# Arcadia-Science/arcadia-microscopy-tools

Measured on AMD Instinct MI355X. Metric: fields-of-view/sec (4x2048^2 uint16) end-to-end segment+props, higher is better.
Workload: dtype f64; 1 GPU; configs[2]: synthetic 4-channel 2048x2048 uint16 FOVs, DAPI Gaussian+Otsu+open/close+EDT+peak markers+watershed nuclei (SEEDED relief, seeds_first: marker pixels spread first in raster order, cannot tie; SURVEY A.8's plain -EDT relief with exact ties is reported under sublines.a8_exact) + clear_border/relabel + morphology and 4-channel intensity regionprops; mode=weak scaling, 192 FOVs per GPU per step, streams_per_gpu=4, fovs_per_launch=48, max_cells_per_fov=2048, distinct_fovs_per_gpu=8, resident_in_hbm=True

## Files before the change

arcadia_microscopy_tools_amd/_thresholds.py:

```python
from __future__ import annotations

import numpy as np
from scipy import ndimage as ndi


def counts_centers_u16(hist65536: np.ndarray):
    nz = np.flatnonzero(hist65536)
    lo, hi = int(nz[0]), int(nz[-1])
    return hist65536[lo:hi + 1].astype(np.int64), np.arange(lo, hi + 1)


def counts_centers_f64(hist: np.ndarray, vmin: float, vmax: float):
    edges = np.linspace(vmin, vmax, len(hist) + 1)
    return hist.astype(np.int64), (edges[:-1] + edges[1:]) / 2.0


def otsu(counts, bin_centers):
    counts = counts.astype(float)
    if len(bin_centers) == 1:
        return bin_centers[0]
    w_lo = np.cumsum(counts)
    w_hi = np.cumsum(counts[::-1])[::-1]
    weighted = counts * bin_centers
    m_lo = np.cumsum(weighted) / w_lo
# ... 52 lines not shown
    length = peak_height * x1 - width * y1
    arg_level = np.argmax(length) + arg_low_level
    if flip:
        arg_level = nbins - arg_level - 1
    return bin_centers[arg_level]


def minimum(counts, bin_centers, max_iter: int = 10000):

    def local_maxima(h):
        step = np.diff(h)
        nz = np.flatnonzero(step)
        if nz.size == 0:
            return []
        falling = step[nz] < 0
        prev_rising = np.ones(nz.size, bool)
        prev_rising[1:] = ~falling[:-1]
        return nz[falling & prev_rising].tolist()

    smooth = counts.astype(np.float64, copy=False)
    maxima: list[int] = []
    counter = 0
    for counter in range(max_iter):
        smooth = ndi.uniform_filter1d(smooth, 3)
        maxima = local_maxima(smooth)
        if len(maxima) < 3:
            break
    if len(maxima) != 2:
        raise RuntimeError("Unable to find two maxima in histogram")
    elif counter == max_iter - 1:
        raise RuntimeError("Maximum iteration reached for histogram smoothing")
    k = np.argmin(smooth[maxima[0]:maxima[1] + 1])
    return bin_centers[maxima[0] + k]


def mean_from_hist(counts, values):
    return float(np.sum(counts * values)) / float(np.sum(counts))


def li_from_hist(counts, values, tolerance=None, initial_guess=None, wrap_dtype=None):
    values = values.astype(np.int64)
    counts = np.asarray(counts)
    image_min = int(values[0])
    v = values - image_min
    if wrap_dtype is not None and np.dtype(wrap_dtype).kind == "i" and int(v[-1]) > int(np.iinfo(wrap_dtype).max):
        half = int(np.iinfo(wrap_dtype).max) + 1
        v = (v + half) % (2 * half) - half
        order = np.argsort(v, kind="stable")
        v, counts = v[order], counts[order]
    present = v[counts > 0]
    if present.size == 1:
        return values[0]
    tolerance = tolerance or np.min(np.diff(present)) / 2
    total_sum = np.sum(counts * v)
    total_cnt = np.sum(counts)
    t_next = total_sum / total_cnt if initial_guess is None else initial_guess - image_min
    t_curr = -2 * tolerance
    csum = np.cumsum(counts * v)
    ccnt = np.cumsum(counts)
    with np.errstate(invalid="ignore", divide="ignore"):
        while abs(t_next - t_curr) > tolerance:
            t_curr = t_next
            k = int(np.searchsorted(v, t_curr, side="right")) - 1
            s_le = csum[k] if k >= 0 else 0
            c_le = ccnt[k] if k >= 0 else 0
            mean_back = np.float64(s_le) / np.float64(c_le)
            mean_fore = np.float64(total_sum - s_le) / np.float64(total_cnt - c_le)
            t_next = (mean_back - mean_fore) / (np.log(mean_back) - np.log(mean_fore))
    return t_next + image_min


def prefix_rule(v: np.ndarray, vmin: float, vmax: float, nbins: int = 256):
    v = np.ascontiguousarray(v, dtype=np.float64)
    if (v < 0).any():
        raise ValueError("the prefix order holds for non-negative samples only")
    hi32 = v.view(np.uint64) >> np.uint64(32) << np.uint64(32)
    vlo, vhi = hi32.view(np.float64), (hi32 | np.uint64(0xFFFFFFFF)).view(np.float64)
    edges = np.linspace(vmin, vmax, nbins + 1)
    bins = np.clip(np.searchsorted(edges, vlo, side="right") - 1, 0, nbins - 1)
    centres = (edges[:-1] + edges[1:]) / 2.0
    above = vlo > centres[bins]
    undecided = ((bins < nbins - 1) & (vhi >= edges[bins + 1])) | (~above & (vhi > centres[bins]))
    return bins, above, undecided
```

arcadia_microscopy_tools_amd/csrc/amt_filters.hip:

```cpp
#include "amt_internal.h"

template <typename TIn>
__device__ __forceinline__ double load_as_f64(const TIn* p, size_t i, double scale);
template <>
__device__ __forceinline__ double load_as_f64<uint16_t>(const uint16_t* p, size_t i, double scale) {
    return (double)p[i] * scale;
}
template <>
__device__ __forceinline__ double load_as_f64<double>(const double* p, size_t i, double scale) {
    return p[i];
}

template <typename TIn>
__device__ __forceinline__ double cvt_f64(TIn v, double scale);
template <>
__device__ __forceinline__ double cvt_f64<uint16_t>(uint16_t v, double scale) {
    return (double)v * scale;
}
template <>
__device__ __forceinline__ double cvt_f64<double>(double v, double scale) {
    return v;
}

template <typename F>
// ... 879 lines not shown

__global__ void convert_u16_f64_kernel(const uint16_t* __restrict__ in, double scale, double* __restrict__ out,
                                       size_t n) {
    size_t i = (size_t)blockIdx.x * blockDim.x + threadIdx.x;
    size_t stride = (size_t)gridDim.x * blockDim.x;
    for (; i < n; i += stride) out[i] = (double)in[i] * scale;
}

__global__ void copy_f64_kernel(const double* __restrict__ in, double* __restrict__ out, size_t n) {
    size_t i = (size_t)blockIdx.x * blockDim.x + threadIdx.x;
    size_t stride = (size_t)gridDim.x * blockDim.x;
    for (; i < n; i += stride) out[i] = in[i];
}

extern "C" int amt_convert_u16_f64(amt_ctx* ctx, const uint16_t* in, double scale, double* out, size_t n) {
    AMT_TRY(amt_set_device(ctx));
    AMT_REQUIRE(in && out, "convert_u16_f64: null pointer");
    if (n == 0) return AMT_OK;
    hipLaunchKernelGGL(convert_u16_f64_kernel, dim3(amt_grid_for(n, 256)), dim3(256), 0, ctx->stream, in, scale, out,
                       n);
    AMT_LAUNCH_CHECK();
    return AMT_OK;
}

extern "C" int amt_gaussian(amt_ctx* ctx, const void* in, int in_dtype, double scale, double* out, int nplanes, int H,
                            int W, const double* weights, int radius, int mode, double cval, size_t in_plane_stride,
                            double* minmax_dev) {
    AMT_TRY(amt_set_device(ctx));
    AMT_TRY(check_gauss_args(in, in_dtype, out, nplanes, H, W, weights, radius));
    AMT_REQUIRE(in_plane_stride == 0 || in_plane_stride >= (size_t)H * W, "gaussian: in_plane_stride smaller than a plane");
    AMT_REQUIRE(radius > 0 || in_plane_stride == 0 || in_plane_stride == (size_t)H * W,
                "gaussian: strided input needs radius >= 1");
    if (nplanes == 0) return AMT_OK;
    size_t n = (size_t)nplanes * H * W;
    if (radius == 0) {
        if (in_dtype == AMT_U16) {
            AMT_TRY(amt_convert_u16_f64(ctx, (const uint16_t*)in, scale, out, n));
        } else {
            hipLaunchKernelGGL(copy_f64_kernel, dim3(amt_grid_for(n, 256)), dim3(256), 0, ctx->stream,
                               (const double*)in, out, n);
            AMT_LAUNCH_CHECK();
        }
        if (minmax_dev) {
            amt_scratch s(ctx);
            amt_buf<unsigned long long> keys(s, (size_t)2 * nplanes);
            AMT_TRY(s.commit());
            AMT_TRY(amt_i_minmax_f64(ctx, out, keys, minmax_dev, nplanes, (size_t)H * W));
        }
        return AMT_OK;
    }
    amt_scratch s(ctx);
    amt_buf<double> wdev(s, 2 * radius + 1);
    amt_buf<double> tmp(s, n, radius > FR_MAX);
    amt_buf<unsigned long long> keys(s, (size_t)2 * nplanes, minmax_dev != nullptr);
    AMT_TRY(s.commit());
    AMT_TRY(amt_param_upload(ctx, wdev, weights, (2 * radius + 1) * sizeof(double)));
    if (!minmax_dev)
        return gaussian_dispatch(ctx, in, in_dtype, scale, out, tmp, nplanes, H, W, wdev, radius, mode, cval,
                                 in_plane_stride);
    if (radius > FR_MAX) {
        AMT_TRY(gaussian_dispatch(ctx, in, in_dtype, scale, out, tmp, nplanes, H, W, wdev, radius, mode, cval,
                                  in_plane_stride));
        return amt_i_minmax_f64(ctx, out, keys, minmax_dev, nplanes, (size_t)H * W);
    }
    AMT_TRY(amt_i_minmax_init(ctx, keys, nplanes));
    AMT_TRY(gaussian_dispatch(ctx, in, in_dtype, scale, out, tmp, nplanes, H, W, wdev, radius, mode, cval,
                              in_plane_stride, keys));
    return amt_i_minmax_finish(ctx, keys, minmax_dev, nplanes);
}


__device__ __forceinline__ double gl_edge(double lo, double hi, double step, int i) {
    return i == GL_NBINS ? hi : (double)i * step + lo;
}

__device__ __forceinline__ int gl_bin(double v, double lo, double hi, double step, double norm) {
    int b = (int)((v - lo) * norm);
    b = b < 0 ? 0 : (b > GL_NBINS - 1 ? GL_NBINS - 1 : b);
    while (b > 0 && v < gl_edge(lo, hi, step, b)) --b;
    while (b < GL_NBINS - 1 && v >= gl_edge(lo, hi, step, b + 1)) ++b;
    return b;
}

__global__ void __launch_bounds__(256) prefix_codes_kernel(const uint32_t* __restrict__ prefix,
                                                           const double* __restrict__ minmax,
                                                           uint32_t* __restrict__ hist, uint16_t* __restrict__ codes,
                                                           size_t n, uint32_t* __restrict__ und_count,
                                                           uint32_t* __restrict__ und_list) {
    __shared__ uint32_t lh[4 * GL_NBINS];
    const int plane = blockIdx.y;
    const int lane = threadIdx.x & 63;
    const double lo = minmax[2 * plane], hi = minmax[2 * plane + 1];
    const uint32_t* src = prefix + (size_t)plane * n;
    uint16_t* dst = codes + (size_t)plane * n;
    const size_t first = ((size_t)blockIdx.x * 256 + threadIdx.x) * 4, stride = (size_t)gridDim.x * 1024;
    if (!(lo < hi)) {
        for (size_t i0 = first; i0 < n; i0 += stride) *reinterpret_cast<uint2*>(dst + i0) = make_uint2(0u, 0u);
        return;
    }
    for (int i = threadIdx.x; i < 4 * GL_NBINS; i += 256) lh[i] = 0;
    __syncthreads();
    uint32_t* mine = lh + (threadIdx.x >> 6) * GL_NBINS;
    const double step = (hi - lo) / (double)GL_NBINS, norm = (double)GL_NBINS / (hi - lo);
    uint32_t* cnt = und_count + (size_t)plane * PFX_CNT_STRIDE;
    uint32_t* list = und_list + (size_t)plane * PFX_CAP;
    bool dead = false;
    for (size_t i0 = first; i0 < n && !dead; i0 += stride) {
        const uint4 p4 = *reinterpret_cast<const uint4*>(src + i0);
        const unsigned p[4] = {p4.x, p4.y, p4.z, p4.w};
        int b4[4];
        double elo4[4], ehi4[4];
#pragma unroll
        for (int u = 0; u < 4; ++u) {
            const double vlo = __hiloint2double((int)p[u], 0);
            int b = (int)((vlo - lo) * norm);
            b = b < 0 ? 0 : (b > GL_NBINS - 1 ? GL_NBINS - 1 : b);
            b4[u] = b;
            elo4[u] = (double)b * step + lo;
            ehi4[u] = gl_edge(lo, hi, step, b + 1);
        }
        unsigned cd[4], undm = 0;
#pragma unroll
        for (int u = 0; u < 4; ++u) {
            const double vlo = __hiloint2double((int)p[u], 0), vhi = __hiloint2double((int)p[u], (int)0xffffffffu);
            int b = b4[u];
            if (vlo < elo4[u] || (b < GL_NBINS - 1 && vlo >= ehi4[u])) {
                b = gl_bin(vlo, lo, hi, step, norm);
                elo4[u] = gl_edge(lo, hi, step, b);
                ehi4[u] = gl_edge(lo, hi, step, b + 1);
            }
            const double ctr = (elo4[u] + ehi4[u]) / 2.0;
            const bool gt = vlo > ctr;
            const bool und = (b < GL_NBINS - 1 && vhi >= ehi4[u]) || (!gt && vhi > ctr);
            undm |= (und ? 1u : 0u) << u;
            cd[u] = und ? 0u : (((unsigned)b << 1) | (gt ? 1u : 0u));
            const unsigned long long act = __ballot(!und);
            if (!act) continue;
            const int l0 = __ffsll((long long)act) - 1;
            const int b0 = __shfl(b, l0);
            const unsigned long long s0 = __ballot(!und && b == b0);
            if (lane == l0) atomicAdd(&mine[b0], (unsigned)__popcll(s0));
            unsigned long long rest = act & ~s0;
            if (rest) {
                const int l1 = __ffsll((long long)rest) - 1;
                const int b1 = __shfl(b, l1);
                const unsigned long long s1 = __ballot(!und && b == b1);
                if (lane == l1) atomicAdd(&mine[b1], (unsigned)__popcll(s1));
                rest &= ~s1;
                if ((rest >> lane) & 1ull) atomicAdd(&mine[b], 1u);
            }
        }
        *reinterpret_cast<uint2*>(dst + i0) = make_uint2(cd[0] | (cd[1] << 16), cd[2] | (cd[3] << 16));
        const unsigned long long any = __ballot(undm != 0);
        if (any) {
            const unsigned long long m0 = __ballot(undm & 1u), m1 = __ballot(undm & 2u), m2 = __ballot(undm & 4u),
                                     m3 = __ballot(undm & 8u);
            const unsigned n0 = __popcll(m0), n1 = __popcll(m1), n2 = __popcll(m2), n3 = __popcll(m3);
            const int leader = __ffsll((long long)any) - 1;
            unsigned base = 0;
            if (lane == leader) base = atomicAdd(cnt, n0 + n1 + n2 + n3);
            base = __shfl(base, leader);
            const unsigned long long below = (1ull << lane) - 1ull;
            const unsigned pos[4] = {base + (unsigned)__popcll(m0 & below), base + n0 + (unsigned)__popcll(m1 & below),
                                     base + n0 + n1 + (unsigned)__popcll(m2 & below),
                                     base + n0 + n1 + n2 + (unsigned)__popcll(m3 & below)};
#pragma unroll
            for (int u = 0; u < 4; ++u)
                if (((undm >> u) & 1u) && pos[u] < PFX_CAP) list[pos[u]] = (uint32_t)(i0 + u);
            dead = base + n0 + n1 + n2 + n3 > PFX_CAP;
        }
    }
    __syncthreads();
    uint32_t* gh = hist + (size_t)plane * GL_NBINS;
    for (int i = threadIdx.x; i < GL_NBINS; i += 256) {
        const uint32_t c = lh[i] + lh[GL_NBINS + i] + lh[2 * GL_NBINS + i] + lh[3 * GL_NBINS + i];
        if (c) atomicAdd(&gh[i], c);
    }
}

constexpr int PFX_FIX_BLOCKS = 64;
template <int R>
__global__ void __launch_bounds__(64) prefix_fixup_kernel(const uint16_t* __restrict__ in, double scale, int H, int W,
                                                          const double* __restrict__ wts, int mode, size_t in_stride,
                                                          const double* __restrict__ minmax,
                                                          const uint32_t* __restrict__ und_count,
                                                          const uint32_t* __restrict__ und_list,
                                                          uint32_t* __restrict__ hist, uint16_t* __restrict__ codes) {
    constexpr int K = 2 * R + 1;
    static_assert(K <= 32, "one half wave per sample");
    __shared__ double cs[2][32];
    const int plane = blockIdx.y;
    const uint32_t cnt = und_count[(size_t)plane * PFX_CNT_STRIDE];
    uint32_t* gh = hist + (size_t)plane * GL_NBINS;
    if (cnt > PFX_CAP) {
        if (blockIdx.x == 0)
            for (int i = threadIdx.x; i < GL_NBINS; i += 64) gh[i] = 0;
        return;
    }
    if (blockIdx.x * 2u >= cnt) return;
    double w[R + 1];
#pragma unroll
    for (int j = 0; j <= R; ++j) w[j] = wts[R - j];
    const uint16_t* src = in + (size_t)plane * in_stride;
    const double lo = minmax[2 * plane], hi = minmax[2 * plane + 1];
    const double step = (hi - lo) / (double)GL_NBINS, norm = (double)GL_NBINS / (hi - lo);
    const int half = threadIdx.x >> 5, d = threadIdx.x & 31;
    for (uint32_t e0 = blockIdx.x * 2u; e0 < cnt; e0 += 2u * PFX_FIX_BLOCKS) {
        const bool valid = e0 + half < cnt;
        const uint32_t idx = valid ? und_list[(size_t)plane * PFX_CAP + e0 + half] : 0u;
        const int y = (int)(idx / (uint32_t)W), x = (int)(idx % (uint32_t)W);
        if (valid && d < K) cs[half][d] = gauss_column<R>(src, scale, H, W, mode, y, x - R + d, w);
        __syncthreads();
        if (valid && d == 0) {
            double c[K];
#pragma unroll
            for (int k = 0; k < K; ++k) c[k] = cs[half][k];
            const double v = gauss_taps<R>(&c[R], w);
            const int b = gl_bin(v, lo, hi, step, norm);
            const double ctr = (gl_edge(lo, hi, step, b) + gl_edge(lo, hi, step, b + 1)) / 2.0;
            atomicAdd(&gh[b], 1u);
            codes[(size_t)plane * H * W + idx] = (uint16_t)((b << 1) | (v > ctr ? 1 : 0));
        }
        __syncthreads();
    }
}

template <int R>
static int launch_codes(amt_ctx* ctx, const uint16_t* in, double scale, int nplanes, int H, int W, const double* wdev,
                        int mode, size_t in_stride, unsigned long long* keys, double* mm, uint32_t* hist,
                        uint16_t* codes, uint32_t* prefix, uint32_t* und_count, uint32_t* und_list) {
    constexpr int RP = (R + 7) & ~7;
    constexpr int OUTW2 = 256 - 2 * RP;
    const int gx2 = (W + OUTW2 - 1) / OUTW2;
    int TH2 = 256;
    while (TH2 > 32 && (long long)gx2 * ((H + TH2 - 1) / TH2) * nplanes < 4LL * ctx->num_cus) TH2 >>= 1;
    dim3 grid2(gx2, (H + TH2 - 1) / TH2, nplanes);
    AMT_TRY(amt_i_minmax_init(ctx, keys, nplanes));
    if (prefix) {
        hipLaunchKernelGGL((gauss_lds_kernel<R, 3>), grid2, dim3(256), 0, ctx->stream, in, scale, (double*)nullptr, H, W,
                           wdev, mode, in_stride, TH2, keys, (const double*)nullptr, (uint32_t*)nullptr,
                           (uint16_t*)nullptr, prefix, (const uint32_t*)nullptr);
        AMT_LAUNCH_CHECK();
        AMT_TRY(amt_i_minmax_finish(ctx, keys, mm, nplanes));
        AMT_HIP_CHECK(hipMemsetAsync(hist, 0, (size_t)nplanes * GL_NBINS * sizeof(uint32_t), ctx->stream));
        AMT_HIP_CHECK(hipMemsetAsync(und_count, 0, (size_t)nplanes * PFX_CNT_STRIDE * sizeof(uint32_t), ctx->stream));
        const size_t n = (size_t)H * W;
        hipLaunchKernelGGL(prefix_codes_kernel, dim3(amt_grid_for(n, 256 * 16, 512), nplanes), dim3(256), 0, ctx->stream,
                           (const uint32_t*)prefix, (const double*)mm, hist, codes, n, und_count, und_list);
        AMT_LAUNCH_CHECK();
        hipLaunchKernelGGL((prefix_fixup_kernel<R>), dim3(PFX_FIX_BLOCKS, nplanes), dim3(64), 0, ctx->stream, in, scale, H, W,
                           wdev, mode, in_stride, (const double*)mm, (const uint32_t*)und_count,
                           (const uint32_t*)und_list, hist, codes);
        AMT_LAUNCH_CHECK();
        hipLaunchKernelGGL((gauss_lds_kernel<R, 2>), grid2, dim3(256), 0, ctx->stream, in, scale, (double*)nullptr, H, W,
                           wdev, mode, in_stride, TH2, (unsigned long long*)nullptr, (const double*)mm, hist, codes,
                           (uint32_t*)nullptr, (const uint32_t*)und_count);
        AMT_LAUNCH_CHECK();
        return AMT_OK;
    }
    hipLaunchKernelGGL((gauss_lds_kernel<R, 1>), grid2, dim3(256), 0, ctx->stream, in, scale, (double*)nullptr, H, W,
                       wdev, mode, in_stride, TH2, keys, (const double*)nullptr, (uint32_t*)nullptr, (uint16_t*)nullptr,
                       (uint32_t*)nullptr, (const uint32_t*)nullptr);
    AMT_LAUNCH_CHECK();
    AMT_TRY(amt_i_minmax_finish(ctx, keys, mm, nplanes));
    AMT_HIP_CHECK(hipMemsetAsync(hist, 0, (size_t)nplanes * GL_NBINS * sizeof(uint32_t), ctx->stream));
    hipLaunchKernelGGL((gauss_lds_kernel<R, 2>), grid2, dim3(256), 0, ctx->stream, in, scale, (double*)nullptr, H, W,
                       wdev, mode, in_stride, TH2, (unsigned long long*)nullptr, (const double*)mm, hist, codes,
                       (uint32_t*)nullptr, (const uint32_t*)nullptr);
    AMT_LAUNCH_CHECK();
    return AMT_OK;
}

extern "C" int amt_gaussian_otsu_codes_supported(int H, int W, int radius, int mode, size_t in_plane_stride) {
    const bool modeok = mode == AMT_MODE_NEAREST || mode == AMT_MODE_REFLECT || mode == AMT_MODE_MIRROR;
    return radius >= 1 && radius <= FR_MAX && modeok && W % 8 == 0 && W >= 256 && H > 2 * radius &&
           (in_plane_stride == 0 || in_plane_stride % 8 == 0);
}

extern "C" int amt_gaussian_otsu_codes(amt_ctx* ctx, const uint16_t* in, double scale, int nplanes, int H, int W,
                                       const double* weights, int radius, int mode, size_t in_plane_stride,
                                       double* minmax_dev, uint32_t* hist_dev, double* thr_dev, double* thr_code_dev,
                                       uint16_t* codes, uint32_t* prefix) {
    AMT_TRY(amt_set_device(ctx));
    AMT_REQUIRE(in && weights && minmax_dev && hist_dev && thr_dev && thr_code_dev && codes && nplanes >= 0,
                "gaussian_otsu_codes: bad arguments");
    AMT_REQUIRE(amt_gaussian_otsu_codes_supported(H, W, radius, mode, in_plane_stride) &&
                    (reinterpret_cast<uintptr_t>(in) & 15) == 0 && (reinterpret_cast<uintptr_t>(codes) & 15) == 0 &&
                    (reinterpret_cast<uintptr_t>(prefix) & 15) == 0,
                "gaussian_otsu_codes: unsupported shape / radius / mode / alignment (ask "
                "amt_gaussian_otsu_codes_supported; the separate operators handle every case)");
    if (nplanes == 0) return AMT_OK;
    if (in_plane_stride == 0) in_plane_stride = (size_t)H * W;
    bool ordered = scale > 0.0 && (size_t)H * W <= 0xffffffffull;
    for (int i = 0; i <= 2 * radius; ++i) ordered = ordered && weights[i] >= 0.0;
    if (!ordered) prefix = nullptr;
    amt_scratch s(ctx);
    amt_buf<double> wdev(s, 2 * radius + 1);
    amt_buf<unsigned long long> keys(s, (size_t)2 * nplanes);
    amt_buf<uint32_t> und_count(s, (size_t)nplanes * PFX_CNT_STRIDE, prefix != nullptr);
    amt_buf<uint32_t> und_list(s, (size_t)nplanes * PFX_CAP, prefix != nullptr);
    AMT_TRY(s.commit());
    AMT_TRY(amt_param_upload(ctx, wdev, weights, (2 * radius + 1) * sizeof(double)));
    switch (radius) {
#define AMT_CODES_CASE(RR)                                                                                            \
    case RR:                                                                                                          \
        AMT_TRY(launch_codes<RR>(ctx, in, scale, nplanes, H, W, wdev, mode, in_plane_stride, keys, minmax_dev, hist_dev, \
                                 codes, prefix, und_count, und_list));                                                \
        break;
        AMT_CODES_CASE(1)
        AMT_CODES_CASE(2)
        AMT_CODES_CASE(3)
        AMT_CODES_CASE(4)
        AMT_CODES_CASE(5)
        AMT_CODES_CASE(6)
        AMT_CODES_CASE(7)
        AMT_CODES_CASE(8)
        AMT_CODES_CASE(9)
        AMT_CODES_CASE(10)
        AMT_CODES_CASE(11)
        AMT_CODES_CASE(12)
#undef AMT_CODES_CASE
        default:
            amt_set_error("gaussian_otsu_codes: radius %d", radius);
            return AMT_EINVAL;
    }
    return amt_i_otsu_from_hist(ctx, hist_dev, minmax_dev, GL_NBINS, thr_dev, thr_code_dev, nplanes);
}

__global__ void sub_inplace_kernel(double* __restrict__ a, const double* __restrict__ b, size_t n) {
    size_t i = (size_t)blockIdx.x * blockDim.x + threadIdx.x;
    size_t stride = (size_t)gridDim.x * blockDim.x;
    for (; i < n; i += stride) a[i] = a[i] - b[i];
}

extern "C" int amt_convolve_axis0(amt_ctx* ctx, const void* in, int in_dtype, double scale, double* out, int nplanes, int L,
                                  int inner, const double* weights, int radius, int mode, double cval) {
    AMT_TRY(amt_set_device(ctx));
    AMT_TRY(check_gauss_args(in, in_dtype, out, nplanes, L, inner, weights, radius));
    AMT_REQUIRE(radius >= 1, "convolve_axis0: radius must be >= 1");
    AMT_REQUIRE((const void*)in != (const void*)out, "convolve_axis0: in-place operation is not supported");
    if (nplanes == 0) return AMT_OK;
    const int r = radius;
// ... 232 lines not shown
```

arcadia_microscopy_tools_amd/csrc/amt_internal.h:

```cpp
#pragma once
#include "amt_common.h"

#include <type_traits>

template <int ITEMS>
__global__ void __launch_bounds__(1024) amt_scan_excl_kernel(int* __restrict__ data, int len, size_t plane_stride,
                                                             int* __restrict__ total,
                                                             const int* __restrict__ len_dev = nullptr) {
    __shared__ int s[1024];
    __shared__ int carry;
    int* d = data + (size_t)blockIdx.x * plane_stride;
    if (len_dev) len = len_dev[blockIdx.x];
    if (threadIdx.x == 0) carry = 0;
    __syncthreads();
    for (int start = 0; start < len; start += 1024 * ITEMS) {
        const int b = start + threadIdx.x * ITEMS;
        int v[ITEMS];
        int sum = 0;
#pragma unroll
        for (int k = 0; k < ITEMS; ++k) {
            v[k] = (b + k < len) ? d[b + k] : 0;
            sum += v[k];
        }
        s[threadIdx.x] = sum;
        __syncthreads();
        for (int off = 1; off < 1024; off <<= 1) {
            int t = threadIdx.x >= off ? s[threadIdx.x - off] : 0;
            __syncthreads();
            s[threadIdx.x] += t;
            __syncthreads();
        }
        const int c = carry;
        int run = c + s[threadIdx.x] - sum;
#pragma unroll
        for (int k = 0; k < ITEMS; ++k) {
            if (b + k < len) d[b + k] = run;
            run += v[k];
        }
        __syncthreads();
        if (threadIdx.x == 1023) carry = c + s[1023];
        __syncthreads();
    }
    if (threadIdx.x == 0 && total) total[blockIdx.x] = carry;
}

static inline int amt_scan_excl(amt_ctx* ctx, int* data, int len, size_t plane_stride, int* total, int nplanes) {
    if (len <= 4096)
        hipLaunchKernelGGL((amt_scan_excl_kernel<4>), dim3(nplanes), dim3(1024), 0, ctx->stream, data, len,
                           plane_stride, total, (const int*)nullptr);
    else
        hipLaunchKernelGGL((amt_scan_excl_kernel<16>), dim3(nplanes), dim3(1024), 0, ctx->stream, data, len,
                           plane_stride, total, (const int*)nullptr);
    AMT_LAUNCH_CHECK();
    return AMT_OK;
}

static inline int amt_scan_excl_dev(amt_ctx* ctx, int* data, const int* len_dev, size_t plane_stride, int* total,
                                    int nplanes) {
    hipLaunchKernelGGL((amt_scan_excl_kernel<8>), dim3(nplanes), dim3(1024), 0, ctx->stream, data, 0, plane_stride,
                       total, len_dev);
    AMT_LAUNCH_CHECK();
    return AMT_OK;
}

int amt_i_minmax_init(amt_ctx* ctx, unsigned long long* keys, int nplanes);
int amt_i_minmax_finish(amt_ctx* ctx, const unsigned long long* keys, double* out, int nplanes);
int amt_i_minmax_f64(amt_ctx* ctx, const double* in, unsigned long long* keys, double* out, int nplanes, size_t n);
int amt_i_otsu_from_hist(amt_ctx* ctx, const uint32_t* hist, const double* minmax, int nbins, double* thr,
                         double* thr_code, int nplanes);

struct ccl_geom {
    int nplanes, H, W;
    size_t n;
    int segs, trows;
    size_t ntiles;
    size_t cap, nlist;
    int nblk;
    int nrow_blocks;
    int jobs;
    dim3 gs;
    dim3 gb;
    dim3 gseams;
    dim3 glists;
    size_t multi_ints() const { return 16 + ntiles * 4; }
};
ccl_geom amt_i_ccl_geom(int nplanes, int H, int W);
int amt_i_ccl_tileroots_u8(amt_ctx* ctx, const ccl_geom& g, const uint8_t* in, int* L, int* rootlist, int* nroots,
                           int* multi = nullptr);
constexpr int RT_CAP = 2048;
static inline bool amt_i_ccl_runs_ok(const void* in, const ccl_geom& g) {
    return g.W % 16 == 0 && (reinterpret_cast<uintptr_t>(in) & 15) == 0 && g.n % 16 == 0;
}
int amt_i_ccl_tileroots_runs_u8(amt_ctx* ctx, const ccl_geom& g, const uint8_t* in, int* L, int* rootlist, int* nroots,
                                unsigned long long* tbits, unsigned short* rtab, int* nruns, unsigned short* roff);
struct amt_runtabs {
    const unsigned long long* tbits;
    const unsigned short* roff;
    const unsigned short* rtab;
    const int* rcomp;
    int segs, trows;
};
int amt_i_propagate_roots(amt_ctx* ctx, const ccl_geom& g, int* A, const int* L, const int* rootlist, const int* nroots);

template <typename F>
static inline void amt_with_bool(bool b, F&& f) {
    if (b) f(std::true_type{});
    else f(std::false_type{});
}

#ifdef __HIPCC__
__device__ __forceinline__ int uf_find_volatile(int* L, int a) {
    int p = __hip_atomic_load(&L[a], __ATOMIC_RELAXED, __HIP_MEMORY_SCOPE_AGENT);
    while (p != a) {
        a = p;
        p = __hip_atomic_load(&L[a], __ATOMIC_RELAXED, __HIP_MEMORY_SCOPE_AGENT);
    }
    return a;
}

__device__ __forceinline__ void uf_union(int* L, int a, int b) {
    while (true) {
        a = uf_find_volatile(L, a);
        b = uf_find_volatile(L, b);
        if (a == b) return;
        if (a < b) {
            int t = a;
            a = b;
            b = t;
        }
        int old = atomicMin(&L[a], b);
        if (old == a) return;
        a = old;
    }
}

__device__ __forceinline__ int lds_find(int* S, int a) {
    int p = __hip_atomic_load(&S[a], __ATOMIC_RELAXED, __HIP_MEMORY_SCOPE_WORKGROUP);
    while (p != a) {
        a = p;
        p = __hip_atomic_load(&S[a], __ATOMIC_RELAXED, __HIP_MEMORY_SCOPE_WORKGROUP);
    }
    return a;
}

__device__ __forceinline__ void lds_union(int* S, int a, int b) {
    while (true) {
        a = lds_find(S, a);
        b = lds_find(S, b);
// ... 51 lines not shown
```

arcadia_microscopy_tools_amd/csrc/amt_stats.hip:

```cpp
#include "amt_common.h"

constexpr int HIST_LDS_BINS = 32768;

__global__ void __launch_bounds__(1024) hist_u16_kernel(const uint16_t* __restrict__ in, uint32_t* __restrict__ hist,
                                                        size_t n, int blocks_per_plane) {
    extern __shared__ __attribute__((aligned(16))) char smem_raw[];
    uint32_t* lh = reinterpret_cast<uint32_t*>(smem_raw);
    const int plane = blockIdx.x / blocks_per_plane;
    const int part = blockIdx.x - plane * blocks_per_plane;
    const uint16_t* src = in + (size_t)plane * n;
    uint32_t* gh = hist + (size_t)plane * 65536;
    const size_t nvec = ((reinterpret_cast<uintptr_t>(src) & 15) == 0) ? n / 8 : 0;
    const uint4* v4 = reinterpret_cast<const uint4*>(src);
    const size_t per = (nvec + blocks_per_plane - 1) / blocks_per_plane;
    const size_t v0 = (size_t)part * per, v1 = v0 + per < nvec ? v0 + per : nvec;
    for (unsigned win = 0; win < 2; ++win) {
        for (int i = threadIdx.x; i < HIST_LDS_BINS; i += 1024) lh[i] = 0;
        __syncthreads();
        unsigned other = 0;
        for (size_t i = v0 + threadIdx.x; i < v1; i += 1024) {
            const uint4 q = v4[i];
            const uint32_t wds[4] = {q.x, q.y, q.z, q.w};
#pragma unroll
            for (int k = 0; k < 4; ++k) {
// ... 37 lines not shown
    for (size_t i = threadIdx.x; i < nvec; i += 1024) {
        const uint4 q = v4[i];
        const uint32_t wds[4] = {q.x, q.y, q.z, q.w};
#pragma unroll
        for (int k = 0; k < 4; ++k) {
            const uint32_t a = wds[k] & 0xffffu, b = wds[k] >> 16;
            atomicAdd(&lh[a >> 1], 1u << ((a & 1u) * 16));
            atomicAdd(&lh[b >> 1], 1u << ((b & 1u) * 16));
        }
    }
    for (size_t i = p0 + nvec * 8 + threadIdx.x; i < p1; i += 1024) {
        const uint32_t a = src[i];
        atomicAdd(&lh[a >> 1], 1u << ((a & 1u) * 16));
    }
    __syncthreads();
    uint4* out = reinterpret_cast<uint4*>(partial + (size_t)blockIdx.x * 32768);
    for (int i = threadIdx.x; i < 8192; i += 1024) out[i] = l4[i];
}

__global__ void __launch_bounds__(256) hist_u16_reduce_kernel(const uint32_t* __restrict__ partial, uint32_t* __restrict__ hist,
                                                              int parts) {
    const int plane = blockIdx.y;
    const int t = blockIdx.x * 256 + threadIdx.x;
    const int w = t >> 2, q = t & 3;
    const uint32_t* p = partial + (size_t)plane * parts * 32768 + w;
    uint32_t lo = 0, hi = 0;
    for (int k = q; k < parts; k += 4) {
        const uint32_t v = p[(size_t)k * 32768];
        lo += v & 0xffffu;
        hi += v >> 16;
    }
    lo += __shfl_xor(lo, 1);
    hi += __shfl_xor(hi, 1);
    lo += __shfl_xor(lo, 2);
    hi += __shfl_xor(hi, 2);
    if (q == 0) reinterpret_cast<uint2*>(hist + (size_t)plane * 65536)[w] = make_uint2(lo, hi);
}

static size_t hist_u16_scratch_bytes(int nplanes, size_t n) {
    if (n == 0 || nplanes <= 0) return 0;
    const size_t parts = (n + HIST_PART_PX - 1) / HIST_PART_PX;
    if (parts * (size_t)nplanes > (size_t)HIST_MAX_PARTS) return 0;
    return amt_align(parts * (size_t)nplanes * 32768 * sizeof(uint32_t));
}

static int hist_u16_launch(amt_ctx* ctx, const uint16_t* in, uint32_t* hist, int nplanes, size_t n,
                           uint32_t* scratch = nullptr) {
    if (n == 0) {
        AMT_HIP_CHECK(hipMemsetAsync(hist, 0, (size_t)nplanes * 65536 * sizeof(uint32_t), ctx->stream));
        return AMT_OK;
    }
    if (scratch && hist_u16_scratch_bytes(nplanes, n) > 0) {
        const int parts = (int)((n + HIST_PART_PX - 1) / HIST_PART_PX);
        hipLaunchKernelGGL(hist_u16_part_kernel, dim3(nplanes * parts), dim3(1024), 32768 * sizeof(uint32_t), ctx->stream, in,
                           scratch, n, parts);
        AMT_LAUNCH_CHECK();
        hipLaunchKernelGGL(hist_u16_reduce_kernel, dim3(512, nplanes), dim3(256), 0, ctx->stream, scratch, hist, parts);
        AMT_LAUNCH_CHECK();
        return AMT_OK;
    }
    AMT_HIP_CHECK(hipMemsetAsync(hist, 0, (size_t)nplanes * 65536 * sizeof(uint32_t), ctx->stream));
    int bpp = (int)((n + 262143) / 262144);
    int cap = (2 * ctx->num_cus + nplanes - 1) / nplanes;
    if (cap < 1) cap = 1;
    if (bpp > cap) bpp = cap;
    if (bpp < 1) bpp = 1;
    hipLaunchKernelGGL(hist_u16_kernel, dim3(nplanes * bpp), dim3(1024), HIST_LDS_BINS * sizeof(uint32_t), ctx->stream,
                       in, hist, n, bpp);
    AMT_LAUNCH_CHECK();
    return AMT_OK;
}

extern "C" int amt_hist_u16(amt_ctx* ctx, const uint16_t* in, uint32_t* hist, int nplanes, size_t n) {
    AMT_TRY(amt_set_device(ctx));
    AMT_REQUIRE(in && hist && nplanes >= 0, "hist_u16: bad arguments");
    if (nplanes == 0) return AMT_OK;
    const size_t sb = hist_u16_scratch_bytes(nplanes, n);
    amt_scratch s(ctx);
    amt_buf<uint32_t> scratch(s, sb / sizeof(uint32_t), sb > 0);
    if (sb) AMT_TRY(s.commit());
    return hist_u16_launch(ctx, in, hist, nplanes, n, scratch);
}

__global__ void minmax_init_kernel(unsigned long long* keys, int nplanes) {
    int i = blockIdx.x * blockDim.x + threadIdx.x;
    if (i < nplanes) {
        keys[2 * i] = ~0ull;
        keys[2 * i + 1] = 0ull;
    }
}

__global__ void __launch_bounds__(256) minmax_f64_kernel(const double* __restrict__ in,
                                                         unsigned long long* __restrict__ keys, size_t n) {
    const int plane = blockIdx.y;
    const double* src = in + (size_t)plane * n;
    unsigned long long lo = ~0ull, hi = 0ull;
    for (size_t i = (size_t)blockIdx.x * 256 + threadIdx.x; i < n; i += (size_t)gridDim.x * 256) {
        unsigned long long k = amt_f64_key(src[i]);
        lo = k < lo ? k : lo;
        hi = k > hi ? k : hi;
    }
#pragma unroll
    for (int off = 32; off >= 1; off >>= 1) {
        unsigned long long l2 = __shfl_xor(lo, off), h2 = __shfl_xor(hi, off);
        lo = l2 < lo ? l2 : lo;
        hi = h2 > hi ? h2 : hi;
    }
    __shared__ unsigned long long s_lo[4], s_hi[4];
    if ((threadIdx.x & 63) == 0) {
        s_lo[threadIdx.x >> 6] = lo;
        s_hi[threadIdx.x >> 6] = hi;
    }
    __syncthreads();
    if (threadIdx.x == 0) {
        for (int k = 1; k < 4; ++k) {
            lo = s_lo[k] < lo ? s_lo[k] : lo;
            hi = s_hi[k] > hi ? s_hi[k] : hi;
        }
        atomicMin(&keys[2 * plane], lo);
        atomicMax(&keys[2 * plane + 1], hi);
    }
}

__global__ void minmax_finish_kernel(const unsigned long long* keys, double* out, int nplanes) {
    int i = blockIdx.x * blockDim.x + threadIdx.x;
    if (i < 2 * nplanes) out[i] = amt_key_f64(keys[i]);
}

int amt_i_minmax_init(amt_ctx* ctx, unsigned long long* keys, int nplanes) {
    hipLaunchKernelGGL(minmax_init_kernel, dim3((nplanes + 63) / 64), dim3(64), 0, ctx->stream, keys, nplanes);
    AMT_LAUNCH_CHECK();
    return AMT_OK;
}

int amt_i_minmax_finish(amt_ctx* ctx, const unsigned long long* keys, double* out, int nplanes) {
    hipLaunchKernelGGL(minmax_finish_kernel, dim3((2 * nplanes + 63) / 64), dim3(64), 0, ctx->stream, keys, out,
                       nplanes);
    AMT_LAUNCH_CHECK();
    return AMT_OK;
}

static int minmax_f64_launch(amt_ctx* ctx, const double* in, unsigned long long* keys, double* out, int nplanes,
                             size_t n) {
    hipLaunchKernelGGL(minmax_init_kernel, dim3((nplanes + 63) / 64), dim3(64), 0, ctx->stream, keys, nplanes);
    AMT_LAUNCH_CHECK();
    if (n) {
        dim3 grid(amt_grid_for(n, 256 * 16, 256), nplanes);
        hipLaunchKernelGGL(minmax_f64_kernel, grid, dim3(256), 0, ctx->stream, in, keys, n);
        AMT_LAUNCH_CHECK();
    }
    hipLaunchKernelGGL(minmax_finish_kernel, dim3((2 * nplanes + 63) / 64), dim3(64), 0, ctx->stream, keys, out,
                       nplanes);
    AMT_LAUNCH_CHECK();
    return AMT_OK;
}

int amt_i_minmax_f64(amt_ctx* ctx, const double* in, unsigned long long* keys, double* out, int nplanes, size_t n) {
    return minmax_f64_launch(ctx, in, keys, out, nplanes, n);
}

extern "C" int amt_minmax_f64(amt_ctx* ctx, const double* in, double* minmax_dev, int nplanes, size_t n) {
    AMT_TRY(amt_set_device(ctx));
    AMT_REQUIRE(in && minmax_dev && nplanes >= 0, "minmax_f64: bad arguments");
    if (nplanes == 0) return AMT_OK;
    amt_scratch s(ctx);
    amt_buf<unsigned long long> keys(s, 2 * nplanes);
    AMT_TRY(s.commit());
    return minmax_f64_launch(ctx, in, keys, minmax_dev, nplanes, n);
}

__device__ __forceinline__ double linspace_edge(double lo, double hi, double step, int i, int nbins) {
    return i == nbins ? hi : (double)i * step + lo;
}

__global__ void __launch_bounds__(256) hist_f64_kernel(const double* __restrict__ in,
                                                       const double* __restrict__ minmax,
                                                       uint32_t* __restrict__ hist, int nbins, size_t n,
                                                       uint8_t* __restrict__ bins) {
    extern __shared__ __attribute__((aligned(16))) char smem_raw[];
    double* edges = reinterpret_cast<double*>(smem_raw);
    uint32_t* lh = reinterpret_cast<uint32_t*>(edges + nbins + 1);
    const int plane = blockIdx.y;
    const double lo = minmax[2 * plane], hi = minmax[2 * plane + 1];
    const double step = (hi - lo) / (double)nbins;
    for (int i = threadIdx.x; i <= nbins; i += 256) edges[i] = linspace_edge(lo, hi, step, i, nbins);
    for (int i = threadIdx.x; i < 4 * nbins; i += 256) lh[i] = 0;
    __syncthreads();
    uint32_t* mine = lh + (threadIdx.x >> 6) * nbins;
    const double norm = (double)nbins / (hi - lo);
    const bool flat = !(lo < hi);
    const double* src = in + (size_t)plane * n;
    const int lane = threadIdx.x & 63;
    const bool vec = (n & 3) == 0 && (reinterpret_cast<uintptr_t>(src) & 31) == 0;
    for (size_t i0 = ((size_t)blockIdx.x * 256 + threadIdx.x) * 4; i0 < n; i0 += (size_t)gridDim.x * 1024) {
        double v4[4];
        if (vec) {
            const double2 a = *reinterpret_cast<const double2*>(src + i0), c = *reinterpret_cast<const double2*>(src + i0 + 2);
            v4[0] = a.x, v4[1] = a.y, v4[2] = c.x, v4[3] = c.y;
        } else {
#pragma unroll
            for (int u = 0; u < 4; ++u) v4[u] = (i0 + u < n) ? src[i0 + u] : __builtin_nan("");
        }
        int b4[4];
        double elo4[4], ehi4[4];
#pragma unroll
        for (int u = 0; u < 4; ++u) {
            const double v = v4[u];
            const bool ok = v >= lo && v <= hi;
            int b = ok ? (flat ? nbins / 2 : (int)((v - lo) * norm)) : 0;
            b = b < 0 ? 0 : (b > nbins - 1 ? nbins - 1 : b);
            b4[u] = b;
            elo4[u] = (double)b * step + lo;
            ehi4[u] = b + 1 == nbins ? hi : (double)(b + 1) * step + lo;
        }
        unsigned packed = 0;
#pragma unroll
        for (int u = 0; u < 4; ++u) {
            const double v = v4[u];
            const bool ok = v >= lo && v <= hi;
            int b = b4[u];
            if (ok && !flat && (v < elo4[u] || (b < nbins - 1 && v >= ehi4[u]))) {
                while (b > 0 && v < edges[b]) --b;
                while (b < nbins - 1 && v >= edges[b + 1]) ++b;
            }
            packed |= (unsigned)(ok && !flat ? b : 0) << (8 * u);
            const unsigned long long act = __ballot(ok);
            if (!act) continue;
// ... 1314 lines not shown
```

Measured before the change: 15630 FOV/s.

## Classify prefix codes via integer LDS tables and merge memsets into init kernel

Each block now precomputes a per-bin table of 32-bit thresholds in LDS (edge start, upper edge, centre bounds). Pixels are then classified with integer compares instead of f64 edge and centre arithmetic, and the histogram ballot aggregation is restructured across the four unrolled pixels. The next uint4 of prefixes is loaded one iteration ahead. The two hipMemsetAsync calls for hist and und_count are folded into the minmax init kernel, which removes launches. The cost is extra LDS, register pressure and more intricate ballot logic that must match the f64 rule exactly.

```diff
diff --git a/arcadia_microscopy_tools_amd/_thresholds.py b/arcadia_microscopy_tools_amd/_thresholds.py
--- a/arcadia_microscopy_tools_amd/_thresholds.py
+++ b/arcadia_microscopy_tools_amd/_thresholds.py
@@ -158,3 +158,30 @@
     above = vlo > centres[bins]
     undecided = ((bins < nbins - 1) & (vhi >= edges[bins + 1])) | (~above & (vhi > centres[bins]))
     return bins, above, undecided
+
+
+def prefix_rule_tables(vmin: float, vmax: float, nbins: int = 256) -> np.ndarray:
+    edges = np.linspace(vmin, vmax, nbins + 1)
+    if (edges < 0).any():
+        raise ValueError("the prefix order holds for non-negative thresholds only")
+    centres = (edges[:-1] + edges[1:]) / 2.0
+    eb, cb = edges.view(np.uint64), centres.view(np.uint64)
+    eh, el = eb >> np.uint64(32), eb & np.uint64(0xFFFFFFFF)
+    ch, cl = cb >> np.uint64(32), cb & np.uint64(0xFFFFFFFF)
+    t = np.full((nbins + 1, 4), 0xFFFFFFFF, np.uint64)
+    t[:nbins, 0] = eh[:nbins] + (el[:nbins] != 0)
+    t[0, 0] = 0
+    t[:nbins - 1, 1] = eh[1:nbins]
+    t[:nbins, 2] = ch + np.uint64(1)
+    t[:nbins, 3] = ch + (cl == np.uint64(0xFFFFFFFF))
+    return t.astype(np.uint32)
+
+
+def prefix_classify(p: np.ndarray, tables: np.ndarray):
+    p = np.asarray(p, dtype=np.uint32)
+    nbins = len(tables) - 1
+    bins = np.clip(np.searchsorted(tables[:nbins, 0], p, side="right") - 1, 0, nbins - 1)
+    row = tables[bins]
+    above = p >= row[..., 2]
+    undecided = (p >= row[..., 1]) | (~above & (p >= row[..., 3]))
+    return bins, above, undecided
diff --git a/arcadia_microscopy_tools_amd/csrc/amt_filters.hip b/arcadia_microscopy_tools_amd/csrc/amt_filters.hip
--- a/arcadia_microscopy_tools_amd/csrc/amt_filters.hip
+++ b/arcadia_microscopy_tools_amd/csrc/amt_filters.hip
@@ -985,11 +985,24 @@
     return b;
 }
 
+__device__ __forceinline__ uint4 pfx_row(double lo, double hi, double step, int b) {
+    const double e0 = gl_edge(lo, hi, step, b), e1 = gl_edge(lo, hi, step, b + 1);
+    const double c = (e0 + e1) / 2.0;
+    const uint32_t hc = (uint32_t)__double2hiint(c);
+    uint4 t;
+    t.x = b == 0 ? 0u : (uint32_t)__double2hiint(e0) + (__double2loint(e0) != 0 ? 1u : 0u);
+    t.y = b == GL_NBINS - 1 ? 0xffffffffu : (uint32_t)__double2hiint(e1);
+    t.z = hc + 1u;
+    t.w = hc + ((uint32_t)__double2loint(c) == 0xffffffffu ? 1u : 0u);
+    return t;
+}
+
 __global__ void __launch_bounds__(256) prefix_codes_kernel(const uint32_t* __restrict__ prefix,
                                                            const double* __restrict__ minmax,
                                                            uint32_t* __restrict__ hist, uint16_t* __restrict__ codes,
                                                            size_t n, uint32_t* __restrict__ und_count,
                                                            uint32_t* __restrict__ und_list) {
+    __shared__ uint4 tab[GL_NBINS + 1];
     __shared__ uint32_t lh[4 * GL_NBINS];
     const int plane = blockIdx.y;
     const int lane = threadIdx.x & 63;
@@ -1001,63 +1014,85 @@
         for (size_t i0 = first; i0 < n; i0 += stride) *reinterpret_cast<uint2*>(dst + i0) = make_uint2(0u, 0u);
         return;
     }
+    const double step = (hi - lo) / (double)GL_NBINS, norm = (double)GL_NBINS / (hi - lo);
+    uint4 p4 = *reinterpret_cast<const uint4*>(src + (first < n ? first : 0));
     for (int i = threadIdx.x; i < 4 * GL_NBINS; i += 256) lh[i] = 0;
+    tab[threadIdx.x] = pfx_row(lo, hi, step, threadIdx.x);
+    if (threadIdx.x == 0) tab[GL_NBINS] = make_uint4(0xffffffffu, 0xffffffffu, 0xffffffffu, 0xffffffffu);
     __syncthreads();
     uint32_t* mine = lh + (threadIdx.x >> 6) * GL_NBINS;
-    const double step = (hi - lo) / (double)GL_NBINS, norm = (double)GL_NBINS / (hi - lo);
     uint32_t* cnt = und_count + (size_t)plane * PFX_CNT_STRIDE;
     uint32_t* list = und_list + (size_t)plane * PFX_CAP;
     bool dead = false;
+    asm volatile("" : "+v"(p4.x), "+v"(p4.y), "+v"(p4.z), "+v"(p4.w));
     for (size_t i0 = first; i0 < n && !dead; i0 += stride) {
-        const uint4 p4 = *reinterpret_cast<const uint4*>(src + i0);
         const unsigned p[4] = {p4.x, p4.y, p4.z, p4.w};
-        int b4[4];
-        double elo4[4], ehi4[4];
+        if (i0 + stride < n) p4 = *reinterpret_cast<const uint4*>(src + i0 + stride);
+        int b[4];
+        uint4 t[4];
+        bool ok[4];
 #pragma unroll
         for (int u = 0; u < 4; ++u) {
             const double vlo = __hiloint2double((int)p[u], 0);
-            int b = (int)((vlo - lo) * norm);
-            b = b < 0 ? 0 : (b > GL_NBINS - 1 ? GL_NBINS - 1 : b);
-            b4[u] = b;
-            elo4[u] = (double)b * step + lo;
-            ehi4[u] = gl_edge(lo, hi, step, b + 1);
-        }
-        unsigned cd[4], undm = 0;
+            int g = (int)((vlo - lo) * norm);
+            g = g < 0 ? 0 : (g > GL_NBINS - 1 ? GL_NBINS - 1 : g);
+            b[u] = g;
+            t[u] = tab[g];
+            ok[u] = p[u] - t[u].x < tab[g + 1].x - t[u].x;
+        }
+        if (!(ok[0] & ok[1] & ok[2] & ok[3])) {
+#pragma unroll
+            for (int u = 0; u < 4; ++u)
+                if (!ok[u]) {
+                    int bb = b[u];
+                    while (bb > 0 && p[u] < tab[bb].x) --bb;
+                    while (bb < GL_NBINS - 1 && p[u] >= tab[bb + 1].x) ++bb;
+                    b[u] = bb;
+                    t[u] = tab[bb];
+                }
+        }
+        const unsigned long long ex = __ballot(true);
+        unsigned cd[4];
+        bool und[4], rem[4];
+        unsigned long long undm[4], remm[4];
 #pragma unroll
         for (int u = 0; u < 4; ++u) {
-            const double vlo = __hiloint2double((int)p[u], 0), vhi = __hiloint2double((int)p[u], (int)0xffffffffu);
-            int b = b4[u];
-            if (vlo < elo4[u] || (b < GL_NBINS - 1 && vlo >= ehi4[u])) {
-                b = gl_bin(vlo, lo, hi, step, norm);
-                elo4[u] = gl_edge(lo, hi, step, b);
-                ehi4[u] = gl_edge(lo, hi, step, b + 1);
+            const bool he = p[u] >= t[u].y, gt = p[u] >= t[u].z, uc = p[u] >= t[u].w;
+            und[u] = he | (!gt & uc);
+            undm[u] = __ballot(he) | (~__ballot(gt) & __ballot(uc));
+            cd[u] = und[u] ? 0u : (((unsigned)b[u] << 1) | (gt ? 1u : 0u));
+            rem[u] = !und[u];
+            remm[u] = ex & ~undm[u];
+        }
+        *reinterpret_cast<uint2*>(dst + i0) = make_uint2(cd[0] | (cd[1] << 16), cd[2] | (cd[3] << 16));
+        unsigned long long act = remm[0] | remm[1] | remm[2] | remm[3];
+#pragma unroll
+        for (int round = 0; round < 2; ++round) {
+            if (act) {
+                const int l = __ffsll((long long)act) - 1;
+                const int fb = rem[0] ? b[0] : (rem[1] ? b[1] : (rem[2] ? b[2] : b[3]));
+                const int bl = __builtin_amdgcn_readlane(fb, l);
+                unsigned c = 0;
+#pragma unroll
+                for (int u = 0; u < 4; ++u) {
+                    const bool same = b[u] == bl;
+                    const unsigned long long hit = remm[u] & __ballot(same);
+                    c += (unsigned)__popcll(hit);
+                    remm[u] &= ~hit;
+                    rem[u] = rem[u] & !same;
+                }
+                if (lane == l) atomicAdd(&mine[bl], c);
+                act = remm[0] | remm[1] | remm[2] | remm[3];
             }
-            const double ctr = (elo4[u] + ehi4[u]) / 2.0;
-            const bool gt = vlo > ctr;
-            const bool und = (b < GL_NBINS - 1 && vhi >= ehi4[u]) || (!gt && vhi > ctr);
-            undm |= (und ? 1u : 0u) << u;
-            cd[u] = und ? 0u : (((unsigned)b << 1) | (gt ? 1u : 0u));
-            const unsigned long long act = __ballot(!und);
-            if (!act) continue;
-            const int l0 = __ffsll((long long)act) - 1;
-            const int b0 = __shfl(b, l0);
-            const unsigned long long s0 = __ballot(!und && b == b0);
-            if (lane == l0) atomicAdd(&mine[b0], (unsigned)__popcll(s0));
-            unsigned long long rest = act & ~s0;
-            if (rest) {
-                const int l1 = __ffsll((long long)rest) - 1;
-                const int b1 = __shfl(b, l1);
-                const unsigned long long s1 = __ballot(!und && b == b1);
-                if (lane == l1) atomicAdd(&mine[b1], (unsigned)__popcll(s1));
-                rest &= ~s1;
-                if ((rest >> lane) & 1ull) atomicAdd(&mine[b], 1u);
-            }
-        }
-        *reinterpret_cast<uint2*>(dst + i0) = make_uint2(cd[0] | (cd[1] << 16), cd[2] | (cd[3] << 16));
-        const unsigned long long any = __ballot(undm != 0);
+        }
+        if (act) {
+#pragma unroll
+            for (int u = 0; u < 4; ++u)
+                if (rem[u]) atomicAdd(&mine[b[u]], 1u);
+        }
+        const unsigned long long any = undm[0] | undm[1] | undm[2] | undm[3];
         if (any) {
-            const unsigned long long m0 = __ballot(undm & 1u), m1 = __ballot(undm & 2u), m2 = __ballot(undm & 4u),
-                                     m3 = __ballot(undm & 8u);
+            const unsigned long long m0 = undm[0], m1 = undm[1], m2 = undm[2], m3 = undm[3];
             const unsigned n0 = __popcll(m0), n1 = __popcll(m1), n2 = __popcll(m2), n3 = __popcll(m3);
             const int leader = __ffsll((long long)any) - 1;
             unsigned base = 0;
@@ -1069,7 +1104,7 @@
                                      base + n0 + n1 + n2 + (unsigned)__popcll(m3 & below)};
 #pragma unroll
             for (int u = 0; u < 4; ++u)
-                if (((undm >> u) & 1u) && pos[u] < PFX_CAP) list[pos[u]] = (uint32_t)(i0 + u);
+                if (und[u] && pos[u] < PFX_CAP) list[pos[u]] = (uint32_t)(i0 + u);
             dead = base + n0 + n1 + n2 + n3 > PFX_CAP;
         }
     }
@@ -1138,15 +1173,14 @@
     int TH2 = 256;
     while (TH2 > 32 && (long long)gx2 * ((H + TH2 - 1) / TH2) * nplanes < 4LL * ctx->num_cus) TH2 >>= 1;
     dim3 grid2(gx2, (H + TH2 - 1) / TH2, nplanes);
-    AMT_TRY(amt_i_minmax_init(ctx, keys, nplanes));
     if (prefix) {
+        AMT_TRY(amt_i_minmax_init(ctx, keys, nplanes, hist, (size_t)nplanes * GL_NBINS, und_count,
+                                  (size_t)nplanes * PFX_CNT_STRIDE));
         hipLaunchKernelGGL((gauss_lds_kernel<R, 3>), grid2, dim3(256), 0, ctx->stream, in, scale, (double*)nullptr, H, W,
                            wdev, mode, in_stride, TH2, keys, (const double*)nullptr, (uint32_t*)nullptr,
                            (uint16_t*)nullptr, prefix, (const uint32_t*)nullptr);
         AMT_LAUNCH_CHECK();
         AMT_TRY(amt_i_minmax_finish(ctx, keys, mm, nplanes));
-        AMT_HIP_CHECK(hipMemsetAsync(hist, 0, (size_t)nplanes * GL_NBINS * sizeof(uint32_t), ctx->stream));
-        AMT_HIP_CHECK(hipMemsetAsync(und_count, 0, (size_t)nplanes * PFX_CNT_STRIDE * sizeof(uint32_t), ctx->stream));
         const size_t n = (size_t)H * W;
         hipLaunchKernelGGL(prefix_codes_kernel, dim3(amt_grid_for(n, 256 * 16, 512), nplanes), dim3(256), 0, ctx->stream,
                            (const uint32_t*)prefix, (const double*)mm, hist, codes, n, und_count, und_list);
@@ -1161,6 +1195,7 @@
         AMT_LAUNCH_CHECK();
         return AMT_OK;
     }
+    AMT_TRY(amt_i_minmax_init(ctx, keys, nplanes));
     hipLaunchKernelGGL((gauss_lds_kernel<R, 1>), grid2, dim3(256), 0, ctx->stream, in, scale, (double*)nullptr, H, W,
                        wdev, mode, in_stride, TH2, keys, (const double*)nullptr, (uint32_t*)nullptr, (uint16_t*)nullptr,
                        (uint32_t*)nullptr, (const uint32_t*)nullptr);
diff --git a/arcadia_microscopy_tools_amd/csrc/amt_internal.h b/arcadia_microscopy_tools_amd/csrc/amt_internal.h
--- a/arcadia_microscopy_tools_amd/csrc/amt_internal.h
+++ b/arcadia_microscopy_tools_amd/csrc/amt_internal.h
@@ -63,7 +63,8 @@
     return AMT_OK;
 }
 
-int amt_i_minmax_init(amt_ctx* ctx, unsigned long long* keys, int nplanes);
+int amt_i_minmax_init(amt_ctx* ctx, unsigned long long* keys, int nplanes, uint32_t* zero_a = nullptr, size_t na = 0,
+                      uint32_t* zero_b = nullptr, size_t nb = 0);
 int amt_i_minmax_finish(amt_ctx* ctx, const unsigned long long* keys, double* out, int nplanes);
 int amt_i_minmax_f64(amt_ctx* ctx, const double* in, unsigned long long* keys, double* out, int nplanes, size_t n);
 int amt_i_otsu_from_hist(amt_ctx* ctx, const uint32_t* hist, const double* minmax, int nbins, double* thr,
diff --git a/arcadia_microscopy_tools_amd/csrc/amt_stats.hip b/arcadia_microscopy_tools_amd/csrc/amt_stats.hip
--- a/arcadia_microscopy_tools_amd/csrc/amt_stats.hip
+++ b/arcadia_microscopy_tools_amd/csrc/amt_stats.hip
@@ -143,12 +143,15 @@
     return hist_u16_launch(ctx, in, hist, nplanes, n, scratch);
 }
 
-__global__ void minmax_init_kernel(unsigned long long* keys, int nplanes) {
-    int i = blockIdx.x * blockDim.x + threadIdx.x;
-    if (i < nplanes) {
-        keys[2 * i] = ~0ull;
-        keys[2 * i + 1] = 0ull;
-    }
+__global__ void minmax_init_kernel(unsigned long long* keys, int nplanes, uint32_t* zero_a, size_t na, uint32_t* zero_b,
+                                   size_t nb) {
+    const size_t i = (size_t)blockIdx.x * blockDim.x + threadIdx.x, step = (size_t)gridDim.x * blockDim.x;
+    for (size_t j = i; j < (size_t)nplanes; j += step) {
+        keys[2 * j] = ~0ull;
+        keys[2 * j + 1] = 0ull;
+    }
+    for (size_t j = i; j < na; j += step) zero_a[j] = 0u;
+    for (size_t j = i; j < nb; j += step) zero_b[j] = 0u;
 }
 
 __global__ void __launch_bounds__(256) minmax_f64_kernel(const double* __restrict__ in,
@@ -188,8 +191,12 @@
     if (i < 2 * nplanes) out[i] = amt_key_f64(keys[i]);
 }
 
-int amt_i_minmax_init(amt_ctx* ctx, unsigned long long* keys, int nplanes) {
-    hipLaunchKernelGGL(minmax_init_kernel, dim3((nplanes + 63) / 64), dim3(64), 0, ctx->stream, keys, nplanes);
+int amt_i_minmax_init(amt_ctx* ctx, unsigned long long* keys, int nplanes, uint32_t* zero_a, size_t na,
+                      uint32_t* zero_b, size_t nb) {
+    const size_t most = na > nb ? na : nb;
+    const size_t want = most > (size_t)nplanes ? most : (size_t)nplanes;
+    const unsigned blocks = (unsigned)((want + 63) / 64 < 1024 ? (want + 63) / 64 : 1024);
+    hipLaunchKernelGGL(minmax_init_kernel, dim3(blocks), dim3(64), 0, ctx->stream, keys, nplanes, zero_a, na, zero_b, nb);
     AMT_LAUNCH_CHECK();
     return AMT_OK;
 }
@@ -203,7 +210,8 @@
 
 static int minmax_f64_launch(amt_ctx* ctx, const double* in, unsigned long long* keys, double* out, int nplanes,
                              size_t n) {
-    hipLaunchKernelGGL(minmax_init_kernel, dim3((nplanes + 63) / 64), dim3(64), 0, ctx->stream, keys, nplanes);
+    hipLaunchKernelGGL(minmax_init_kernel, dim3((nplanes + 63) / 64), dim3(64), 0, ctx->stream, keys, nplanes,
+                       (uint32_t*)nullptr, (size_t)0, (uint32_t*)nullptr, (size_t)0);
     AMT_LAUNCH_CHECK();
     if (n) {
         dim3 grid(amt_grid_for(n, 256 * 16, 256), nplanes);
```

Result: faster. 16160 FOV/s (median of 6 runs) (+3.4%).
